# sjpollard/video-how-do-your-tokens-merge

Hardware: AMD Instinct MI355X
Metric: clips/sec at r=16, VideoMAE-B 16x224x224 (forward with ToMe merge; merge indices bit-exact against the fp32-arithmetic oracle, which the reference's fp32 fixtures pin) (higher is better)
Workload: dtype bf16; 1 GPU; VideoMAE-B random-init, synthetic 16x224x224 clips, r=16, bf16 (BASELINE.json configs[1]); r=16, parallelism=dp1: independent replicas, one RCCL all-reduce of [top1, top5, clips], step_launch=eager

## Files before the change

### video-how-do-your-tokens-merge_amd/csrc/tome_attn_stream.h

```cpp
#pragma once
#include "tome_attn.h"

#ifdef ATT_DIAG
#define ATS_STAMP(i)                                                                                       \
    do {                                                                                                   \
        if (diag_n == 2 && blockIdx.x < ATT_DIAG_WGS) {                                                    \
            const unsigned long long st_ = __builtin_amdgcn_s_memrealtime();                               \
            if (lane == 0) g_att_stamps[((size_t)blockIdx.x * 8 + wave) * ATT_DIAG_N + (i)] = st_;          \
        }                                                                                                  \
    } while (0)
#else
#define ATS_STAMP(i)
#endif

#define ATS_BIAS_GROUP 4
template <typename TX, bool BIAS>
__global__ __launch_bounds__(512, 2) void k_prop_attention_stream(AttnArgs a, int nitems) {
    constexpr int WAVES = 8;
    constexpr int ATT_BM = 32 * WAVES;
    __shared__ __attribute__((aligned(16))) short lds_k[ATT_SLOTS][ATT_BN * ATT_KS];
    __shared__ __attribute__((aligned(16))) short lds_v[ATT_SLOTS][ATT_BN * ATT_VS];
    __shared__ __attribute__((aligned(16))) unsigned lds_bias[2][ATS_BIAS_GROUP * ATT_BN];
    __shared__ __attribute__((aligned(16))) short lds_o[WAVES][32 * ATT_KS];

    const int tid = threadIdx.x, lane = tid & 63, wave = __builtin_amdgcn_readfirstlane(tid >> 6);

    const int col = lane & 31, hf = lane >> 5;
    const int qblocks = (a.N + ATT_BM - 1) / ATT_BM;
    const int nbhs = a.B * a.H * a.nseg;
    const int G = gridDim.x;
    const int ntiles = (a.Nk + ATT_BN - 1) / ATT_BN;
    const int nfull = a.Nk / ATT_BN;
    const bool last_half = (ntiles - 1) * ATT_BN + 32 >= a.Nk;
    const float LOG2E = 1.4426950408889634f;
    const float sl = a.scale * LOG2E;
    typedef const __attribute__((address_space(4))) AttnArgs *AttnArgsK;
    const AttnArgsK kargs = (AttnArgsK)__builtin_amdgcn_kernarg_segment_ptr();
    auto fresh = [&]() __attribute__((always_inline)) -> AttnArgsK {
        AttnArgsK p = kargs;
        asm volatile("" : "+s"(p));
        return p;
    };
    const int nseg = a.nseg, nheads = a.H, nq = a.N, nk = a.Nk, bias_skip = a.bias_skip;
    const int64_t k_tile = (int64_t)ATT_BN * a.k_sn * 2, v_tile = (int64_t)ATT_BN * a.v_sn * 2;

    struct Item { int b, h, seg, qb; };
    auto item_ok = [&](int L) -> bool {
        if (L >= nitems) return false;
        const int sq = L >> 3;
        return (sq / qblocks) * 8 + (L & 7) < nbhs;
    };
    auto decode = [&](int L) -> Item {
        const int sq = L >> 3;
        const int bhs = (sq / qblocks) * 8 + (L & 7);
        Item it;
        it.qb = sq % qblocks;
        const int bh = bhs / nseg;
        it.seg = bhs - bh * nseg;
        it.b = bh / nheads;
        it.h = bh % nheads;
        return it;
    };

    const int r0 = tid >> 3, c0 = tid & 7;
    const int rp = min(r0, max(nk - nfull * ATT_BN, 1) - 1);
    const unsigned koff = (unsigned)(((int64_t)r0 * a.k_sn + 8 * c0) * 2), koff_p = (unsigned)(((int64_t)rp * a.k_sn + 8 * c0) * 2);
    const unsigned voff = (unsigned)(((int64_t)r0 * a.v_sn + 8 * c0) * 2), voff_p = (unsigned)(((int64_t)rp * a.v_sn + 8 * c0) * 2);
    uint4 kreg, vreg;
    unsigned breg = 0u;
    int r_sub = 0, b_par = 0, b_off = 0;
    const char *s_kt = nullptr, *s_vt = nullptr;
    const float *s_ls = nullptr;
    int s_t = 0, s_item = 0;
    const short *n_q = nullptr;
    short *n_o = nullptr;
    int n_qb = 0;
    auto stream_set = [&](int L) __attribute__((always_inline)) {
        const Item it = decode(L);
        const AttnArgsK A = fresh();
        s_kt = reinterpret_cast<const char *>(reinterpret_cast<const short *>(A->k) + it.b * A->k_sb + it.h * A->k_sh + it.seg * A->k_seg);
        s_vt = reinterpret_cast<const char *>(reinterpret_cast<const short *>(A->v) + it.b * A->v_sb + it.h * A->v_sh + it.seg * A->v_seg);
        if (BIAS) s_ls = A->log_size + it.b * A->ls_sb + it.seg * A->ls_seg;
        n_q = reinterpret_cast<const short *>(A->q) + it.b * A->q_sb + it.h * A->q_sh + (int64_t)it.qb * ATT_BM * A->q_sn;
        n_o = reinterpret_cast<short *>(A->out) + it.b * A->o_sb + it.h * A->o_sh + it.seg * A->o_seg + (int64_t)it.qb * ATT_BM * A->o_sn;
        n_qb = it.qb;
        s_item = L;
        s_t = 0;
    };
    auto stream_load = [&]() __attribute__((always_inline)) {
        const bool part = s_t >= nfull;
        kreg = *reinterpret_cast<const uint4 *>(s_kt + (part ? koff_p : koff));
        vreg = *reinterpret_cast<const uint4 *>(s_vt + (part ? voff_p : voff));
        r_sub = s_t & (ATS_BIAS_GROUP - 1);
        if (BIAS && r_sub == 0 && tid < ATS_BIAS_GROUP * ATT_BN) {
            const int key = min(s_t * ATT_BN + tid, nk - 1);
            const float bv = key >= bias_skip ? s_ls[key - bias_skip] * LOG2E : 0.0f;
            const short bh = att_bits<TX>(bv);
            TX th;
            __builtin_memcpy(&th, &bh, 2);
            const short bl = att_bits<TX>(bv - to_f32(th));
            breg = (unsigned)(unsigned short)bh | ((unsigned)(unsigned short)bl << 16);
        }
        if (++s_t == ntiles) {
            if (item_ok(s_item + G)) stream_set(s_item + G);
            else s_t = ntiles - 1;
        } else {
            s_kt += k_tile;
            s_vt += v_tile;
        }
    };
    short *const wk = &lds_k[0][0] + r0 * ATT_KS + 8 * c0, *const wv = &lds_v[0][0] + r0 * ATT_VS + 8 * c0;
    auto stage_write = [&](int S) __attribute__((always_inline)) {
        *reinterpret_cast<uint4 *>(wk + S * ATT_BN * ATT_KS) = kreg;
        *reinterpret_cast<uint4 *>(wv + S * ATT_BN * ATT_VS) = vreg;
        if (BIAS) {
            if (r_sub == 0) {
                b_par ^= 1;
                if (tid < ATS_BIAS_GROUP * ATT_BN) lds_bias[b_par][tid] = breg;
            }
            b_off = b_par * (ATS_BIAS_GROUP * ATT_BN) + r_sub * ATT_BN;
        }
    };

    const int lrow0 = wave * 32 + col;
    const int q_sn = (int)a.q_sn, o_sn = (int)a.o_sn;
    int c_qb = 0;
    short *c_o = nullptr;
    int qrow = 0;
    bool active = false;
    float bfac = 1.0f;
    att_s16x8 qf[4];
    uint4 qraw[4];
    int t_qb = 0;
    short *t_o = nullptr;
    auto q_request = [&]() __attribute__((always_inline)) {
        t_qb = n_qb;
        t_o = n_o;
        const int lrow = max(min(lrow0, nq - 1 - t_qb * ATT_BM), 0);
        const short *qp = n_q + lrow * q_sn + 8 * hf;
#pragma unroll
        for (int ks = 0; ks < 4; ++ks) qraw[ks] = *reinterpret_cast<const uint4 *>(qp + 16 * ks);
    };
    auto item_take = [&]() __attribute__((always_inline)) {
        c_qb = t_qb;
        c_o = t_o;
        qrow = c_qb * ATT_BM + lrow0;
        active = c_qb * ATT_BM + wave * 32 < nq;
        bfac = (bias_skip && qrow == 0) ? 0.0f : 1.0f;
    };
    auto q_convert = [&]() __attribute__((always_inline)) {
#pragma unroll
        for (int ks = 0; ks < 4; ++ks) {
            att_s16x8 raw;
            __builtin_memcpy(&raw, &qraw[ks], 16);
#pragma unroll
            for (int e = 0; e < 8; ++e) {
                TX tq;
                const short r = raw[e];
                __builtin_memcpy(&tq, &r, 2);
                qf[ks][e] = att_bits<TX>(to_f32(tq) * sl);
            }
        }
    };

    att_f32x16 o0, o1, negm, s0, s1;
    float m_run = -INFINITY, l_run = 0.0f;
#ifdef ATT_DIAG
    int diag_n = 0;
    unsigned long long diag_wait_stage = 0, diag_wait_barrier = 0;
#endif
    auto item_reset = [&]() __attribute__((always_inline)) {
#pragma unroll
        for (int v = 0; v < 16; ++v) o0[v] = o1[v] = negm[v] = 0.0f;
        m_run = -INFINITY;
        l_run = 0.0f;
    };

    typedef __attribute__((address_space(3))) att_s16x4 *lds_s16x4_p;
    const short *const vbase = &lds_v[0][0] + (4 * hf + ((lane & 15) >> 2)) * ATT_VS + 16 * ((lane >> 4) & 1) + 4 * (lane & 3);
    const short *const kbase = &lds_k[0][0] + col * ATT_KS + 8 * hf;
    att_s16x4 vfr[2][2][4];
    auto v_fragments = [&](int S) __attribute__((always_inline)) {
        const short *vs = vbase + S * ATT_BN * ATT_VS;
#pragma unroll
        for (int kb = 0; kb < 2; ++kb)
#pragma unroll
            for (int p = 0; p < 2; ++p) {
                const short *va = vs + (32 * kb + 16 * p) * ATT_VS;
                vfr[kb][p][0] = __builtin_amdgcn_ds_read_tr16_b64_v4i16((lds_s16x4_p)(va));
                vfr[kb][p][1] = __builtin_amdgcn_ds_read_tr16_b64_v4i16((lds_s16x4_p)(va + 8 * ATT_VS));
                vfr[kb][p][2] = __builtin_amdgcn_ds_read_tr16_b64_v4i16((lds_s16x4_p)(va + 32));
                vfr[kb][p][3] = __builtin_amdgcn_ds_read_tr16_b64_v4i16((lds_s16x4_p)(va + 8 * ATT_VS + 32));
            }
    };
    auto bias_step = [&](int S) __attribute__((always_inline)) {
        const unsigned w0 = lds_bias[0][b_off + col], w1 = lds_bias[0][b_off + 32 + col];
        const unsigned one = (unsigned)(unsigned short)att_bits<TX>(bfac);
        const unsigned qw = hf ? 0u : (one | (one << 16));
        const uint4 q5 = make_uint4(qw, 0u, 0u, 0u), k0 = make_uint4(hf ? 0u : w0, 0u, 0u, 0u), k1 = make_uint4(hf ? 0u : w1, 0u, 0u, 0u);
        att_s16x8 fq, f0, f1;
        __builtin_memcpy(&fq, &q5, 16);
        __builtin_memcpy(&f0, &k0, 16);
        __builtin_memcpy(&f1, &k1, 16);
        s0 = AttMfma<TX>::run(f0, fq, s0);
        s1 = AttMfma<TX>::run(f1, fq, s1);
    };
    auto scores = [&](int S, const att_f32x16 &cinit, bool first_half_only) __attribute__((always_inline)) {
        const short *ks0 = kbase + S * ATT_BN * ATT_KS;
        s0 = cinit;
        s1 = cinit;
        if (BIAS) bias_step(S);
#pragma unroll
        for (int ks = 0; ks < 4; ++ks)
            s0 = AttMfma<TX>::run(*reinterpret_cast<const att_s16x8 *>(ks0 + 16 * ks), qf[ks], s0);
        if (!first_half_only) {
#pragma unroll
            for (int ks = 0; ks < 4; ++ks)
                s1 = AttMfma<TX>::run(*reinterpret_cast<const att_s16x8 *>(ks0 + 32 * ATT_KS + 16 * ks), qf[ks], s1);
        }
    };
    att_s16x8 pf[2][2];
    auto pack_p = [&]() __attribute__((always_inline)) {
#pragma unroll
        for (int p = 0; p < 2; ++p)
#pragma unroll
            for (int e = 0; e < 8; ++e) {
                pf[0][p][e] = att_bits<TX>(s0[8 * p + e]);
                pf[1][p][e] = att_bits<TX>(s1[8 * p + e]);
            }
    };
    auto general_softmax = [&](int t, int S) __attribute__((always_inline)) {
        att_f32x16 zero;
#pragma unroll
        for (int v = 0; v < 16; ++v) zero[v] = 0.0f;
        scores(S, zero, false);
        const int key0 = t * ATT_BN + 4 * hf;
        float mt = -INFINITY;
#pragma unroll
        for (int v = 0; v < 16; ++v) {
            const int key = key0 + (v & 3) + 8 * (v >> 2);
            s0[v] = key < nk ? s0[v] : -INFINITY;
            s1[v] = key + 32 < nk ? s1[v] : -INFINITY;
            mt = fmaxf(mt, fmaxf(s0[v], s1[v]));
        }
        {
            const unsigned mb = __float_as_uint(mt);
            const auto sw = __builtin_amdgcn_permlane32_swap(mb, mb, false, false);
            mt = fmaxf(__uint_as_float(sw[0]), __uint_as_float(sw[1]));
        }
        const float m_new = fmaxf(m_run, mt);
        const float alpha = __builtin_amdgcn_exp2f(m_run - m_new);
        float lsum = 0.0f;
#pragma unroll
        for (int v = 0; v < 16; ++v) {
            s0[v] = __builtin_amdgcn_exp2f(s0[v] - m_new);
            s1[v] = __builtin_amdgcn_exp2f(s1[v] - m_new);
            lsum += s0[v] + s1[v];
        }
        l_run = l_run * alpha + lsum;
        m_run = m_new;
#pragma unroll
        for (int v = 0; v < 16; ++v) {
            o0[v] *= alpha;
            o1[v] *= alpha;
            negm[v] = -m_new;
        }
        pack_p();
    };
    auto first_softmax = [&](int S) __attribute__((always_inline)) {
        att_f32x16 zero;
#pragma unroll
        for (int v = 0; v < 16; ++v) zero[v] = 0.0f;
        scores(S, zero, false);
        float mt = fmaxf(s0[0], s1[0]);
#pragma unroll
        for (int v = 1; v < 16; ++v) mt = fmaxf(mt, fmaxf(s0[v], s1[v]));
        {
            const unsigned mb = __float_as_uint(mt);
            const auto sw = __builtin_amdgcn_permlane32_swap(mb, mb, false, false);
            mt = fmaxf(__uint_as_float(sw[0]), __uint_as_float(sw[1]));
        }
        float lsum = 0.0f;
#pragma unroll
        for (int v = 0; v < 16; ++v) {
            s0[v] = __builtin_amdgcn_exp2f(s0[v] - mt);
            s1[v] = __builtin_amdgcn_exp2f(s1[v] - mt);
            lsum += s0[v] + s1[v];
        }
        l_run = lsum;
        m_run = mt;
#pragma unroll
        for (int v = 0; v < 16; ++v) negm[v] = -mt;
        pack_p();
    };
    auto pv = [&](bool first_half_only) __attribute__((always_inline)) {
#pragma unroll
        for (int kb = 0; kb < 2; ++kb) {
            if (kb == 1 && first_half_only) break;
#pragma unroll
            for (int p = 0; p < 2; ++p) {
                att_s16x8 vf0, vf1;
#pragma unroll
                for (int e = 0; e < 4; ++e) {
                    vf0[e] = vfr[kb][p][0][e];
                    vf0[4 + e] = vfr[kb][p][1][e];
                    vf1[e] = vfr[kb][p][2][e];
                    vf1[4 + e] = vfr[kb][p][3][e];
                }
                o0 = AttMfma<TX>::run(vf0, pf[kb][p], o0);
                o1 = AttMfma<TX>::run(vf1, pf[kb][p], o1);
            }
        }
    };
    auto fast_step = [&](int S, int tn, bool masked) __attribute__((always_inline)) {
#ifdef ATT_DIAG
        unsigned long long d0_ = 0, d1_ = 0, d2_ = 0;
        if (diag_n == 2) d0_ = __builtin_amdgcn_s_memrealtime();
#endif
        stage_write(S);
#ifdef ATT_DIAG
        if (diag_n == 2) {
            asm volatile("s_waitcnt vmcnt(0) lgkmcnt(0)" ::: "memory");
            d1_ = __builtin_amdgcn_s_memrealtime();
        }
#endif
        stream_load();
        __syncthreads();
#ifdef ATT_DIAG
        if (diag_n == 2) {
            d2_ = __builtin_amdgcn_s_memrealtime();
            diag_wait_stage += d1_ - d0_;
            diag_wait_barrier += d2_ - d1_;
        }
#endif
        scores(S, negm, masked && last_half);
        pv(false);
        v_fragments(S);
        __builtin_amdgcn_s_setprio(1);
#pragma unroll
        for (int v = 0; v < 16; ++v) s0[v] = __builtin_amdgcn_exp2f(s0[v]);
#pragma unroll
        for (int v = 0; v < 16; ++v) s1[v] = __builtin_amdgcn_exp2f(s1[v]);
        if (masked) {
            const int key0 = tn * ATT_BN + 4 * hf;
#pragma unroll
            for (int v = 0; v < 16; ++v) {
                const int key = key0 + (v & 3) + 8 * (v >> 2);
                s0[v] = key < nk ? s0[v] : 0.0f;
                s1[v] = key + 32 < nk ? s1[v] : 0.0f;
            }
        }
        float c0s = att_add(s0[0], s0[4]), c1s = att_add(s0[1], s0[5]), c2s = att_add(s0[2], s0[6]),
              c3s = att_add(s0[3], s0[7]);
#pragma unroll
        for (int v = 8; v < 16; v += 4) {
            c0s = att_add(c0s, s0[v]);     c1s = att_add(c1s, s0[v + 1]);
            c2s = att_add(c2s, s0[v + 2]); c3s = att_add(c3s, s0[v + 3]);
        }
#pragma unroll
        for (int v = 0; v < 16; v += 4) {
            c0s = att_add(c0s, s1[v]);     c1s = att_add(c1s, s1[v + 1]);
            c2s = att_add(c2s, s1[v + 2]); c3s = att_add(c3s, s1[v + 3]);
        }
        const float lsum = att_add(att_add(c0s, c1s), att_add(c2s, c3s));
        pack_p();
        __builtin_amdgcn_s_setprio(0);
        const float l_before = l_run;
        l_run += lsum;
#ifndef ATS_NOGUARD
        if (__builtin_amdgcn_ballot_w64(!(lsum <= AttLimit<TX>::value)) != 0) {
            l_run = l_before;
            general_softmax(tn, S);
        }
#endif
    };
    auto helper_step = [&](int S) __attribute__((always_inline)) {
        stage_write(S);
        stream_load();
        __syncthreads();
    };
    auto store_item = [&]() __attribute__((always_inline)) {
        const float l_tot = l_run + __shfl_xor(l_run, 32);
        const float inv = __builtin_amdgcn_rcpf(l_tot);
        short *ow = &lds_o[0][0] + wave * (32 * ATT_KS);
#pragma unroll
        for (int g = 0; g < 4; ++g) {
            att_s16x4 w0, w1;
#pragma unroll
            for (int e = 0; e < 4; ++e) {
                w0[e] = att_bits<TX>(o0[4 * g + e] * inv);
                w1[e] = att_bits<TX>(o1[4 * g + e] * inv);
            }
            unsigned a2[2], b2[2];
            __builtin_memcpy(a2, &w0, 8);
            __builtin_memcpy(b2, &w1, 8);
            const auto s0w = __builtin_amdgcn_permlane32_swap(a2[0], b2[0], false, false);
            const auto s1w = __builtin_amdgcn_permlane32_swap(a2[1], b2[1], false, false);
            *reinterpret_cast<uint4 *>(ow + col * ATT_KS + 32 * hf + 8 * g) = uint4{s0w[0], s1w[0], s0w[1], s1w[1]};
        }
        const int rows = nq - c_qb * ATT_BM - wave * 32;
        short *op = c_o + (wave * 32 + (lane >> 3)) * o_sn + 8 * (lane & 7);
#pragma unroll
        for (int i = 0; i < 4; ++i) {
            const uint4 row16 = *reinterpret_cast<const uint4 *>(ow + ((lane >> 3) + 8 * i) * ATT_KS + 8 * (lane & 7));
            if ((lane >> 3) + 8 * i < rows) *reinterpret_cast<uint4 *>(op + 8 * i * o_sn) = row16;
        }
    };
    auto cold_start = [&](int L) __attribute__((always_inline)) {
        stream_set(L);
        q_request();
        item_take();
        item_reset();
        stream_load();
        q_convert();
        stage_write(0);
        stream_load();
        __syncthreads();
        if (active) {
            first_softmax(0);
            v_fragments(0);
        }
    };

    int item = blockIdx.x;
    if (!item_ok(item)) return;
    cold_start(item);
    int par = 0;
    for (;;) {
        ATS_STAMP(0);
        if (active) {
            int tn = 1;
            for (; tn < nfull; ++tn) fast_step((par + tn) & 1, tn, false);
            if (tn < ntiles) fast_step((par + tn) & 1, tn, true);
        } else {
            for (int tn = 1; tn < ntiles; ++tn) helper_step((par + tn) & 1);
        }
        ATS_STAMP(1);
#ifdef ATT_DIAG
        if (diag_n == 2 && blockIdx.x < ATT_DIAG_WGS && lane == 0) {
            g_att_stamps[((size_t)blockIdx.x * 8 + wave) * ATT_DIAG_N + 6] = diag_wait_stage;
            g_att_stamps[((size_t)blockIdx.x * 8 + wave) * ATT_DIAG_N + 7] = diag_wait_barrier;
        }
#endif
        const int next = item + G;
        const bool has_next = item_ok(next);
        const int Sn = (par + ntiles) & 1;
        if (has_next) {
            stage_write(Sn);
            q_request();
            stream_load();
        }
        const bool was_active = active;
        if (was_active) {
            pv(last_half);
            store_item();
            ATS_STAMP(2);
            if (!has_next) return;
            __syncthreads();
            ATS_STAMP(3);
        } else {
            if (!has_next) return;
            __syncthreads();
        }
        item = next;
        par = Sn;
        item_take();
        item_reset();
        q_convert();
        ATS_STAMP(4);
        if (active) {
            first_softmax(Sn);
            v_fragments(Sn);
        }
        ATS_STAMP(5);
#ifdef ATT_DIAG
        ++diag_n;
#endif
    }
}
```

Before: 2613 clips/s.

## Deepen K/V staging pipeline by one tile and preload K fragments before LDS write

Restructures the streaming attention loop so the barrier comes first, then the staged tile for step t+1 is written into the other LDS slot while the current slot is consumed. In the no-bias path, K fragments are read into registers before that write. The stream load is split into a next-item advance and an issue step, cold start now primes two stages, and the bias offset is delayed by one stage to match. This aims to shorten the wait between the global-load write and the barrier and overlap the LDS writes with MFMA work. In exchange it adds register pressure for the K fragments and makes the slot and bias-offset bookkeeping harder to keep correct.

```diff
diff --git a/video-how-do-your-tokens-merge_amd/csrc/tome_attn_stream.h b/video-how-do-your-tokens-merge_amd/csrc/tome_attn_stream.h
--- a/video-how-do-your-tokens-merge_amd/csrc/tome_attn_stream.h
+++ b/video-how-do-your-tokens-merge_amd/csrc/tome_attn_stream.h
@@ -68,7 +68,7 @@
     const unsigned voff = (unsigned)(((int64_t)r0 * a.v_sn + 8 * c0) * 2), voff_p = (unsigned)(((int64_t)rp * a.v_sn + 8 * c0) * 2);
     uint4 kreg, vreg;
     unsigned breg = 0u;
-    int r_sub = 0, b_par = 0, b_off = 0;
+    int r_sub = 0, b_par = 0, b_off = 0, b_nxt = 0;
     const char *s_kt = nullptr, *s_vt = nullptr;
     const float *s_ls = nullptr;
     int s_t = 0, s_item = 0;
@@ -87,7 +87,13 @@
         s_item = L;
         s_t = 0;
     };
-    auto stream_load = [&]() __attribute__((always_inline)) {
+    auto stream_next = [&]() __attribute__((always_inline)) {
+        if (s_t == ntiles) {
+            if (item_ok(s_item + G)) stream_set(s_item + G);
+            else s_t = ntiles - 1;
+        }
+    };
+    auto stream_issue = [&]() __attribute__((always_inline)) {
         const bool part = s_t >= nfull;
         kreg = *reinterpret_cast<const uint4 *>(s_kt + (part ? koff_p : koff));
         vreg = *reinterpret_cast<const uint4 *>(s_vt + (part ? voff_p : voff));
@@ -101,24 +107,26 @@
             const short bl = att_bits<TX>(bv - to_f32(th));
             breg = (unsigned)(unsigned short)bh | ((unsigned)(unsigned short)bl << 16);
         }
-        if (++s_t == ntiles) {
-            if (item_ok(s_item + G)) stream_set(s_item + G);
-            else s_t = ntiles - 1;
-        } else {
+        if (++s_t < ntiles) {
             s_kt += k_tile;
             s_vt += v_tile;
         }
+    };
+    auto stream_load = [&]() __attribute__((always_inline)) {
+        stream_next();
+        stream_issue();
     };
     short *const wk = &lds_k[0][0] + r0 * ATT_KS + 8 * c0, *const wv = &lds_v[0][0] + r0 * ATT_VS + 8 * c0;
     auto stage_write = [&](int S) __attribute__((always_inline)) {
         *reinterpret_cast<uint4 *>(wk + S * ATT_BN * ATT_KS) = kreg;
         *reinterpret_cast<uint4 *>(wv + S * ATT_BN * ATT_VS) = vreg;
         if (BIAS) {
+            b_off = b_nxt;
             if (r_sub == 0) {
                 b_par ^= 1;
                 if (tid < ATS_BIAS_GROUP * ATT_BN) lds_bias[b_par][tid] = breg;
             }
-            b_off = b_par * (ATS_BIAS_GROUP * ATT_BN) + r_sub * ATT_BN;
+            b_nxt = b_par * (ATS_BIAS_GROUP * ATT_BN) + r_sub * ATT_BN;
         }
     };
 
@@ -219,6 +227,26 @@
                 s1 = AttMfma<TX>::run(*reinterpret_cast<const att_s16x8 *>(ks0 + 32 * ATT_KS + 16 * ks), qf[ks], s1);
         }
     };
+    att_s16x8 kfr[8];
+    auto k_fragments = [&](int S, bool first_half_only) __attribute__((always_inline)) {
+        const short *ks0 = kbase + S * ATT_BN * ATT_KS;
+#pragma unroll
+        for (int ks = 0; ks < 4; ++ks) kfr[ks] = *reinterpret_cast<const att_s16x8 *>(ks0 + 16 * ks);
+        if (!first_half_only) {
+#pragma unroll
+            for (int ks = 0; ks < 4; ++ks) kfr[4 + ks] = *reinterpret_cast<const att_s16x8 *>(ks0 + 32 * ATT_KS + 16 * ks);
+        }
+    };
+    auto scores_mfma = [&](const att_f32x16 &cinit, bool first_half_only) __attribute__((always_inline)) {
+        s0 = cinit;
+        s1 = cinit;
+#pragma unroll
+        for (int ks = 0; ks < 4; ++ks) s0 = AttMfma<TX>::run(kfr[ks], qf[ks], s0);
+        if (!first_half_only) {
+#pragma unroll
+            for (int ks = 0; ks < 4; ++ks) s1 = AttMfma<TX>::run(kfr[4 + ks], qf[ks], s1);
+        }
+    };
     att_s16x8 pf[2][2];
     auto pack_p = [&]() __attribute__((always_inline)) {
 #pragma unroll
@@ -317,23 +345,31 @@
         unsigned long long d0_ = 0, d1_ = 0, d2_ = 0;
         if (diag_n == 2) d0_ = __builtin_amdgcn_s_memrealtime();
 #endif
-        stage_write(S);
+        stream_next();
+        __syncthreads();
+#ifdef ATT_DIAG
+        if (diag_n == 2) d1_ = __builtin_amdgcn_s_memrealtime();
+#endif
+        if (!BIAS) {
+            k_fragments(S, masked && last_half);
+            asm volatile("" ::: "memory");
+        }
+        stage_write(S ^ 1);
 #ifdef ATT_DIAG
         if (diag_n == 2) {
             asm volatile("s_waitcnt vmcnt(0) lgkmcnt(0)" ::: "memory");
-            d1_ = __builtin_amdgcn_s_memrealtime();
-        }
-#endif
-        stream_load();
-        __syncthreads();
-#ifdef ATT_DIAG
-        if (diag_n == 2) {
             d2_ = __builtin_amdgcn_s_memrealtime();
-            diag_wait_stage += d1_ - d0_;
-            diag_wait_barrier += d2_ - d1_;
-        }
-#endif
-        scores(S, negm, masked && last_half);
+            diag_wait_barrier += d1_ - d0_;
+            diag_wait_stage += d2_ - d1_;
+        }
+#endif
+        stream_issue();
+        if (!BIAS) {
+            asm volatile("" ::: "memory");
+            scores_mfma(negm, masked && last_half);
+        } else {
+            scores(S, negm, masked && last_half);
+        }
         pv(false);
         v_fragments(S);
         __builtin_amdgcn_s_setprio(1);
@@ -375,9 +411,10 @@
 #endif
     };
     auto helper_step = [&](int S) __attribute__((always_inline)) {
-        stage_write(S);
-        stream_load();
+        stream_next();
         __syncthreads();
+        stage_write(S ^ 1);
+        stream_issue();
     };
     auto store_item = [&]() __attribute__((always_inline)) {
         const float l_tot = l_run + __shfl_xor(l_run, 32);
@@ -414,6 +451,8 @@
         stream_load();
         q_convert();
         stage_write(0);
+        stream_load();
+        stage_write(1);
         stream_load();
         __syncthreads();
         if (active) {
@@ -445,12 +484,11 @@
         const int next = item + G;
         const bool has_next = item_ok(next);
         const int Sn = (par + ntiles) & 1;
+        const bool was_active = active;
         if (has_next) {
-            stage_write(Sn);
             q_request();
-            stream_load();
-        }
-        const bool was_active = active;
+            stream_next();
+        }
         if (was_active) {
             pv(last_half);
             store_item();
@@ -462,6 +500,8 @@
             if (!has_next) return;
             __syncthreads();
         }
+        stage_write(Sn ^ 1);
+        stream_issue();
         item = next;
         par = Sn;
         item_take();
```

Measured after the change: 2624 clips/s (median of 6 runs). About the same (+0.4%).
